# bodo-ai/Bodo

Measured on NVIDIA H100. Metric: groupby-agg rows/sec, higher is better.
Workload: dtype int64

## Files before the change

bodo_b200/csrc/groupby.cu:

```cuda
#include <algorithm>
#include <chrono>
#include <cmath>
#include <cstdio>
#include <cstdlib>
#include <cstring>
#include <type_traits>
#include <memory>
#include <vector>

#include <cooperative_groups.h>
#include <cooperative_groups/reduce.h>

#include "common.cuh"

namespace b200 {

constexpr long long EMPTY_KEY = (long long)0x8000000000000000ULL;
constexpr int MAX_OPS = 16;
constexpr int64_t CHUNK_ROWS = 1ll << 28;

enum OpKind : int { K_SUM_I64 = 0, K_SUM_F64, K_COUNT, K_SIZE, K_MEAN, K_MIN_I64, K_MAX_I64, K_MIN_F64, K_MAX_F64,
                    K_MOM2, K_MOM3,
                    K_FIRST, K_LAST,
                    K_NUNIQUE,
// ... 1522 lines not shown
    long long* retry_ctr;
    long long retry_cap;
    int sum_first;
    int ns;
    int n_pass;
    const long long* hot_tab;
    const int* n_hot;
    int reserve_tickets;
};
struct SpgDenseArgs : SpgArgs {
    long long kbase, vbase;
    unsigned int d_kb, d_vb;
    unsigned int d_mul, d_inv;
    unsigned int d_gmagic;
    int d_slots;
};

__device__ __forceinline__ uint64_t spg_hash(long long key) {
    uint64_t x = (uint64_t)key;
    return (x ^ (x >> 29)) * 0x9E3779B97F4A7C15ULL;
}
__device__ __forceinline__ unsigned int spg_owner(uint64_t h, int n_owners) { return __umulhi((unsigned int)(h >> 32), (unsigned int)n_owners); }
__device__ __forceinline__ unsigned int spg_slot(uint64_t h, int ns) { return __umulhi((unsigned int)(h >> 20), (unsigned int)ns); }

template <bool HAS_SUM, bool HAS_CNT>
__device__ __forceinline__ void spg_retry_row(const SpgArgs& a, long long key, unsigned long long sum, unsigned long long cnt) {
    unsigned long long f = atomicAdd((unsigned long long*)a.retry_ctr, 1ull);
    if (f >= (unsigned long long)a.retry_cap) { a.counters[CTR_RETRY_OVERFLOW] = 1; return; }
    unsigned long long* r = a.retry + f * 4;
    r[0] = (unsigned long long)key; r[1] = 1ull;
// ... 111 lines not shown
                 ::"r"(smem_u32(smem_dst)), "l"(gsrc), "r"(bytes), "r"(smem_u32(bar)) : "memory");
}

template <int TILE, int MAX_C, int ROW_BYTES, int TAIL>
struct SpgTileSmem {
    static constexpr size_t raw_k = 0, raw_v = raw_k + (size_t)TILE * 8, stage = raw_v + (size_t)TILE * 8;
    static constexpr size_t gbase = stage + (size_t)TILE * ROW_BYTES, mbar = gbase + (size_t)MAX_C * 8, hist = mbar + 16;
    static constexpr size_t lbase = hist + (size_t)MAX_C * 4, tail = lbase + (size_t)(MAX_C + 4) * 4, bytes = tail + TAIL;
    static_assert(stage % 16 == 0 && gbase % 16 == 0 && lbase % 16 == 0 && tail % 16 == 0, "K1 shared regions stay 16-byte aligned");
};

template <int TILE, int THREADS, typename Smem, typename LoadTma, typename LoadPartial, typename Init, typename Classify,
          typename Stage, typename OnRun, typename CopyOut>
__device__ __forceinline__ void spg_partition_tiles(unsigned char* smem, int64_t n_rows, int C, unsigned long long* cls_cnt,
                                                    LoadTma load_tma, LoadPartial load_partial, Init init, Classify classify,
                                                    Stage stage, OnRun on_run, CopyOut copy_out) {
    unsigned long long* gbase = (unsigned long long*)(smem + Smem::gbase);
    uint64_t* mbar = (uint64_t*)(smem + Smem::mbar);
    unsigned int* hist = (unsigned int*)(smem + Smem::hist);
    unsigned int* lbase = (unsigned int*)(smem + Smem::lbase);
    const int tid = threadIdx.x;
    constexpr int ROWS = TILE / THREADS;
    const int64_t n_tiles = (n_rows + TILE - 1) / TILE;
    if (tid == 0) {
        mbar_init(mbar, 1);
        asm volatile("fence.mbarrier_init.release.cluster;" ::: "memory");
        init();
    }
    for (int j = tid; j < C; j += THREADS) hist[j] = 0;
    __syncthreads();
    auto issue = [&](int64_t t) {
        const int64_t r0 = t * TILE;
        if (r0 + TILE <= n_rows && tid == 0) load_tma(r0, mbar);
    };
    uint32_t phase = 0;
    int64_t t = blockIdx.x;
    if (t < n_tiles) issue(t);
    for (; t < n_tiles; t += gridDim.x) {
        const int64_t r0 = t * TILE;
        const int64_t tn = t + gridDim.x;
        const bool full = r0 + TILE <= n_rows;
        if (full) {
            while (!mbar_try_wait(mbar, phase)) {}
            phase ^= 1;
        } else {
            load_partial(r0);
            __syncthreads();
        }
        int c[ROWS];
        unsigned int rk[ROWS];
        [[maybe_unused]] unsigned int w[ROWS];
#pragma unroll
        for (int r = 0; r < ROWS; r++) {
            const int j = r * THREADS + tid;
            c[r] = -1;
// ... 17 lines not shown
            }
            if (tid == 0) lbase[C] = carry;
        }
        __syncthreads();
#pragma unroll
        for (int r = 0; r < ROWS; r++) {
            if (c[r] < 0) continue;
            stage(lbase[c[r]] + rk[r], r * THREADS + tid, c[r], w[r]);
        }
        if (tid >= THREADS - C) {
            const int cl = tid - (THREADS - C);
            gbase[cl] = my_gbase - lbase[cl];
            on_run(cl, my_gbase, my_cnt);
        }
        __syncthreads();
        if (tn < n_tiles) issue(tn);
        copy_out(lbase[C]);
        for (int j = tid; j < C; j += THREADS) hist[j] = 0;
        __syncthreads();
    }
}

template <bool HOT>
using SpgK1Smem = SpgTileSmem<SPG_TILE, SPG_MAX_OWNERS, 16, SPG_TILE + (HOT ? SPG_HOT_SLOTS * 20 : 0)>;

template <bool HAS_SUM, bool HAS_CNT, bool HOT = false>
__global__ void __launch_bounds__(SPG_TTHREADS, SPG_TCTAS) spg_partition_tma_kernel(const __grid_constant__ SpgArgs a) {
    extern __shared__ __align__(128) unsigned char smem_tma_raw[];
    using L = SpgK1Smem<HOT>;
    long long* raw_k = (long long*)(smem_tma_raw + L::raw_k);
    long long* raw_v = (long long*)(smem_tma_raw + L::raw_v);
    longlong2* stage = (longlong2*)(smem_tma_raw + L::stage);
    const unsigned long long* gbase = (const unsigned long long*)(smem_tma_raw + L::gbase);
    unsigned char* stage_owner = smem_tma_raw + L::tail;
// ... 787 lines not shown
        {
            spgn_ns = ((int)(((size_t)max_smem - 256 - SPGN_QUEUE_BYTES) / 12) - SPG_STASH) & ~1;
            spgn_smem = (size_t)(spgn_ns + SPG_STASH) * 12 + SPGN_QUEUE_BYTES + 16;
            spgn_enabled = true;
            spgd_max_smem = (size_t)max_smem - 256;
            for_each_sum_cnt([&](auto s, auto c) {
                if (!set_smem_limit((const void*)spgn_partition_kernel<s, c>, SpgnK1Smem<false>::bytes)) spgn_enabled = false;
                if (!set_smem_limit((const void*)spgn_aggregate_kernel<s, c>, spgn_smem)) spgn_enabled = false;
                if (!set_smem_limit((const void*)spgn_partition_kernel<s, c, true>, SpgnK1Smem<true>::bytes)) spgd_max_smem = 0;
                if (!set_smem_limit((const void*)spgn_aggregate_kernel<s, c, true>, spgd_max_smem)) spgd_max_smem = 0;
            });
            const char* e8 = getenv("B200_SPG_NARROW");
            if (e8 && e8[0] == '0') spgn_enabled = false;
            const char* e9 = getenv("B200_SPG_DENSE");
            if ((e9 && e9[0] == '0') || !spgn_enabled || sms < 2) spgd_max_smem = 0;
        }
        {
            spgg_enabled = 2 * sms <= GEN_CLS;
            for_each_spgg_part([&](auto ks, auto vs) {
                if (!set_smem_limit((const void*)spgg_partition_kernel<ks, vs>, SpggK1Smem::bytes)) spgg_enabled = false;
            });
            for (int v = 0; v < 4; v++) {
                const int sb = 16 + ((v & 1) ? 16 : 0) + ((v & 2) ? 4 : 0);
                spgg_ns[v] = ((int)(((size_t)max_smem - 64) / sb) - SPG_STASH) & ~1;
                spgg_smem[v] = (size_t)(spgg_ns[v] + SPG_STASH) * sb + 16;
            }
            for_each_spgg_agg([&](auto s, auto mm, auto nn) {
                if (!set_smem_limit((const void*)spgg_aggregate_kernel<s, mm, nn>, spgg_smem[mm + 2 * nn])) spgg_enabled = false;
            });
            const char* e7 = getenv("B200_SPG_GEN");
            if (e7 && e7[0] == '0') spgg_enabled = false;
        }
        if (!set_smem_limit((const void*)spg_hot_sample_kernel, SPG_HOT_SAMPLE_SMEM)) return false;
        { const char* e4 = getenv("B200_SPG_HOT"); spg_hot_enabled = !(e4 && e4[0] == '0'); }
        d_hot.alloc((size_t)SPG_HOT_SLOTS * 8 + 48);
        { const char* e3 = getenv("B200_LC"); lc_enabled = !(e3 && e3[0] == '0'); }
        spg_owners = sms;
        d_bucket_cnt.alloc((size_t)(GEN_CLS + spg_owners) * SPG_CNT_STRIDE * 8);
        spg_state = 1;
        return true;
    }

    bool lc_enabled = true, lowcard_small = false;
    int spgn_ns = 0;
    size_t spgn_smem = 0;
    bool spgn_enabled = false;
    int spg_sample_wide = -1;
    int64_t spgn_launches = 0, spg16_launches = 0;
    size_t spgd_max_smem = 0;
    bool spgd_ok = false;
    long long spgd_kbase = 0, spgd_vbase = 0;
    unsigned int spgd_kb = 0, spgd_vb = 0;
    int spgd_slots = 0;
    int64_t spgd_wide_rows = 0, spgd_launches = 0;
    static constexpr unsigned int SPGD_MUL = 0x9E3779B1u;
    static unsigned int odd_inverse(unsigned int m) {
        unsigned int x = m;
        for (int i = 0; i < 4; i++) x *= 2u - m * x;
        return x;
    }
    void spgd_plan(long long kmin, long long kmax, long long vmin, long long vmax, bool has_vals) {
        spgd_ok = false;
        if (spgd_max_smem == 0 || kmin > kmax) return;
        const uint64_t range = (uint64_t)kmax - (uint64_t)kmin;
        if (range >= (1ull << 21)) return;
        const uint64_t pad = range / 32;
        long long kbase;
        if (kmin >= 0 && (uint64_t)kmin <= pad) kbase = 0;
        else if (kmin < LLONG_MIN + (long long)pad + 1) return;
// ... 28 lines not shown
    static constexpr int SPG_MAX_PASSES = 24;
    int spg_pass_count(int64_t est) const {
        int64_t p = (est + spg_group_capacity() - 1) / spg_group_capacity();
        return p <= 1 ? 1 : (p <= SPG_MAX_PASSES ? (int)p : 0);
    }
    bool lc_pick(int64_t est) { lowcard_small = est <= LC_SLOTS_SMALL / 4; return lc_enabled && est <= LC_SLOTS_BIG / 4; }
    int64_t spg_group_capacity() const { return (int64_t)spg_owners * (spg_ns * 7 / 10); }

    PooledBuf d_retry2[2];
    static constexpr int H_SPG_WORDS = 2 * N_COUNTERS + 5;
    long long* h_spg = nullptr;
    cudaEvent_t spg_ev[2] = {nullptr, nullptr};

    int64_t spgn_wide_rows = 0;
    static int spg_retry_slot(int slot) { return slot == 0 ? CTR_FAIL : CTR_RETRY1; }
    void spg_finish(int slot, int sum_j, int cnt_j) {
        B200_CUDA(cudaEventSynchronize(spg_ev[slot]));
        const long long* hc = h_spg + slot * N_COUNTERS;
        n_groups = hc[CTR_GROUPS];
        spgn_wide_rows = hc[CTR_WIDE];
        spgd_wide_rows = hc[CTR_DENSE_WIDE];
        const int64_t nr = hc[spg_retry_slot(slot)];
        if (nr == 0) return;
        spg_retry_rows += nr;
        B200_CUDA(cudaStreamSynchronize(stream));
        read_counters();
        B200_REQUIRE(h_counters[CTR_RETRY_OVERFLOW] == 0, "SM-partitioned groupby: a retry list overflowed its buffer (internal sizing error)");
        const int64_t pending = h_counters[CTR_FAIL] + h_counters[CTR_RETRY1];
        if (pending == 0) return;
        grow_to_fit(pending, (int64_t)spg_owners * spg_ns);
        for (int sl = 0; sl < 2; sl++) {
            int64_t cnt = h_counters[spg_retry_slot(sl)];
            if (cnt == 0) continue;
            B200_CUDA(cudaMemsetAsync((char*)d_counters.p + spg_retry_slot(sl) * 8, 0, 8, stream));
            CombineArgs c{};
            c.src = host_source(d_retry2[sl].p, &cnt, 1); c.row_words = 4;
            d_fail.ensure(device, (size_t)cnt * 4);
            c.fail_list = d_fail.as<uint32_t>(); c.n_ops = 0;
            int order[2] = {sum_j, cnt_j};
            if (sum_j >= 0 && cnt_j >= 0 && cnt_j < sum_j) std::swap(order[0], order[1]);
            if (order[0] < 0) std::swap(order[0], order[1]);
            for (int q = 0; q < 2; q++) if (order[q] >= 0) { c.kinds[c.n_ops] = K_SUM_I64; c.a0[c.n_ops] = d_a0[order[q]].p; c.a1[c.n_ops] = nullptr; c.n_ops++; }
            xchg_combine_kernel<<<grid_for(cnt), 256, 0, stream>>>(slot_table(), c);
            launches++;
            B200_CUDA(cudaGetLastError());
        }
        read_counters();
    }

    void consume_spg(const long long* keys, const long long* vals, int64_t n, int sum_j, int cnt_j, bool lowcard = false, int64_t est_groups = 0) {
        B200_REQUIRE(((uintptr_t)keys & 15) == 0 && ((uintptr_t)vals & 15) == 0, "SM-partitioned groupby: key and value columns must be 16-byte aligned");
        if (!h_spg) {
            h_spg = (long long*)pinned_acquire(H_SPG_WORDS * sizeof(long long));
            for (int b = 0; b < 2; b++) B200_CUDA(cudaEventCreateWithFlags(&spg_ev[b], cudaEventDisableTiming));
        }
        ScopedTimer timer{t_spg};
        read_counters();
        n_groups_bound = n_groups;
        if (!lowcard && !spg_hot_sampled) {
            int* d_nhot = (int*)(d_hot.as<long long>() + SPG_HOT_SLOTS);
            spg_hot_sample_kernel<<<1, 1024, SPG_HOT_SAMPLE_SMEM, stream>>>(keys, vals, n, d_hot.as<long long>(), d_nhot, d_hot.as<long long>() + SPG_HOT_SLOTS + 1);
            B200_CUDA(cudaMemcpyAsync(h_spg + 2 * N_COUNTERS, d_nhot, 5 * sizeof(long long), cudaMemcpyDeviceToHost, stream));
            B200_CUDA(cudaStreamSynchronize(stream));
            spg_n_hot = spg_hot_enabled ? ((int*)(h_spg + 2 * N_COUNTERS))[0] : 0;
            spg_sample_wide = ((int*)(h_spg + 2 * N_COUNTERS))[1];
            const long long* rng = h_spg + 2 * N_COUNTERS + 1;
            spgd_plan(rng[0], rng[1], rng[2], rng[3], vals != nullptr);
            spg_hot_sampled = true;
            launches++;
        }
        const bool narrow_sig = spgn_enabled && !lowcard && spg_n_hot == 0 && spg_sample_wide == 0;
        const int64_t launch_rows = narrow_sig ? 2 * SPG_LAUNCH_ROWS : SPG_LAUNCH_ROWS;
        int64_t li = 0;
        for (int64_t r0 = 0; r0 < n; r0 += launch_rows, li++) {
            int slot = (int)(li & 1);
            int64_t rows = std::min(launch_rows, n - r0);
            const int64_t bucket_cap = (rows / spg_owners) + (rows / spg_owners) / 8 + 4096;
            const bool small = lowcard_small;
            const int gl = (int)std::min<int64_t>((int64_t)sms * (small ? 3 : 2), (rows + LC_THREADS * 2 - 1) / (LC_THREADS * 2));
            const int g2 = (int)std::min<int64_t>((int64_t)sms * SPG_TCTAS, (rows + SPG_TILE - 1) / SPG_TILE);
            const bool hot = !lowcard && spg_hot_enabled && spg_n_hot > 0;
            const bool dense = narrow_sig && spgd_ok && spgd_wide_rows * 64 <= rows_consumed;
            const bool narrow = dense || (narrow_sig && spgn_wide_rows * 64 <= rows_consumed);
            const int64_t est_n = std::max<int64_t>(est_groups, 1);
            const int n_pass = dense ? 1 : narrow ? (int)std::min<int64_t>(SPG_MAX_PASSES, std::max<int64_t>(1, (est_n + spgn_group_capacity() - 1) / spgn_group_capacity()))
                                      : spg_passes;
            const int64_t retry_cap = rows + (lowcard ? (int64_t)gl * (small ? LC_SLOTS_SMALL : LC_SLOTS_BIG)
                                                      : (int64_t)spg_owners * ((narrow ? spgn_ns : spg_ns) + SPG_STASH) * n_pass
                                                        + (hot ? (int64_t)g2 * SPG_HOT_SLOTS : 0));
            double ta = now();
            d_bucket.ensure(device, (size_t)spg_owners * bucket_cap * 16);
            d_retry2[slot].ensure(device, (size_t)retry_cap * 32);
            t_alloc += now() - ta;
            B200_CUDA(cudaMemsetAsync(d_bucket_cnt.p, 0, (size_t)spg_owners * SPG_CNT_STRIDE * 8, stream));
            SpgArgs a{};
            a.keys = keys + r0; a.vals = vals ? vals + r0 : nullptr; a.n_rows = rows; a.n_owners = spg_owners;
            a.tkeys = d_keys.as<long long>(); a.cap = cap;
            a.acc_sum = sum_j >= 0 ? d_a0[sum_j].as<unsigned long long>() : nullptr;
            a.acc_cnt = cnt_j >= 0 ? d_a0[cnt_j].as<unsigned long long>() : nullptr;
            a.counters = d_counters.as<long long>(); a.group_limit = (long long)(cap / 2);
            a.retry_ctr = d_counters.as<long long>() + spg_retry_slot(slot);
            a.bucket = d_bucket.as<longlong2>(); a.bucket_cnt = d_bucket_cnt.as<unsigned long long>(); a.bucket_cap = bucket_cap;
            a.retry = d_retry2[slot].as<unsigned long long>(); a.retry_cap = retry_cap;
            a.sum_first = (sum_j >= 0 && cnt_j >= 0 && sum_j < cnt_j) ? 1 : 0; a.ns = spg_ns; a.n_pass = n_pass;
            const ProfEvents prof = prof_begin(profiling);
            if (lowcard) {
                size_t lsm = (size_t)(small ? LC_SLOTS_SMALL : LC_SLOTS_BIG) * 20 + 64;
                with_sum_cnt(sum_j >= 0, cnt_j >= 0, [&](auto s, auto c) {
                    if (small) groupby_lowcard_kernel<s, c, LC_SLOTS_SMALL, 3><<<gl, LC_THREADS, lsm, stream>>>(a);
                    else groupby_lowcard_kernel<s, c, LC_SLOTS_BIG, 2><<<gl, LC_THREADS, lsm, stream>>>(a);
                });
                lc_launches++;
            } else {
                if (hot) { a.hot_tab = d_hot.as<long long>(); a.n_hot = (const int*)(d_hot.as<long long>() + SPG_HOT_SLOTS); }
                if (narrow) {
                    a.ns = spgn_ns;
                    a.reserve_tickets = (n_groups_bound == 0 && li == 0 && est_groups > 0 && est_groups + est_groups / 4 <= (int64_t)(cap / 2)) ? 1 : 0;
                    a.bucket_cap = bucket_cap & ~1ll;
                    const int gn = (int)std::min<int64_t>((int64_t)sms * SPGN_CTAS, (rows + SPGN_TILE - 1) / SPGN_TILE);
                    if (dense) {
                        a.bucket_cap = bucket_cap & ~3ll;
                        SpgDenseArgs da{};
                        static_cast<SpgArgs&>(da) = a;
                        da.kbase = spgd_kbase; da.vbase = spgd_vbase; da.d_kb = spgd_kb; da.d_vb = spgd_vb;
                        da.d_mul = SPGD_MUL; da.d_inv = odd_inverse(SPGD_MUL);
                        da.d_gmagic = (unsigned int)((0xffffffffull + spg_owners) / spg_owners);
                        da.d_slots = spgd_slots;
                        const size_t dsm = (size_t)spgd_slots * 8;
                        with_sum_cnt(sum_j >= 0, cnt_j >= 0, [&](auto s, auto c) {
                            spgn_partition_kernel<s, c, true><<<gn, SPG_TTHREADS, SpgnK1Smem<true>::bytes, stream>>>(da);
                            spgn_aggregate_kernel<s, c, true><<<spg_owners, SPG_THREADS, dsm, stream>>>(da);
                        });
                        spgd_launches++;
                    } else {
                        with_sum_cnt(sum_j >= 0, cnt_j >= 0, [&](auto s, auto c) {
                            spgn_partition_kernel<s, c><<<gn, SPG_TTHREADS, SpgnK1Smem<false>::bytes, stream>>>(a);
                            spgn_aggregate_kernel<s, c><<<spg_owners, SPG_THREADS, spgn_smem, stream>>>(a);
                        });
                    }
                    spgn_launches++;
                } else {
                    with_sum_cnt(sum_j >= 0, cnt_j >= 0, [&](auto s, auto c) {
                        if (hot) spg_partition_tma_kernel<s, c, true><<<g2, SPG_TTHREADS, SpgK1Smem<true>::bytes, stream>>>(a);
                        else spg_partition_tma_kernel<s, c><<<g2, SPG_TTHREADS, SpgK1Smem<false>::bytes, stream>>>(a);
                        spg_aggregate_kernel<s, c><<<spg_owners, SPG_THREADS, spg_smem, stream>>>(a);
                    });
                    spg16_launches++;
                }
            }
            B200_CUDA(cudaGetLastError());
            prof_end(prof);
            B200_CUDA(cudaMemcpyAsync(h_spg + slot * N_COUNTERS, d_counters.p, N_COUNTERS * sizeof(long long), cudaMemcpyDeviceToHost, stream));
            B200_CUDA(cudaEventRecord(spg_ev[slot], stream));
            launches += 2; consume_launches++; spg_launches++;
            rows_consumed += rows;
            if (li > 0) spg_finish(1 - slot, sum_j, cnt_j);
        }
        if (li > 0) spg_finish((int)((li - 1) & 1), sum_j, cnt_j);
        read_counters();
        n_groups_bound = n_groups;
    }

    struct GenSig { int vcol = -1; bool has_sum = false, has_mm = false, has_nn = false; int layout = 0; };
    static bool gen_int_ok(int ct) { const int sz = ctype_size(ct); return (sz == 4 || sz == 8) && !ctype_is_float(ct) && ct != CT_UINT64; }
    bool gen_signature(const std::vector<const void*>& data, const std::vector<const uint8_t*>& valid, GenSig& gs) const {
        if (nk != 1 || n_funcs < 1 || n_funcs > GEN_MAX_F || !gen_int_ok(c_types[0])) return false;
        bool has_size = false;
        for (auto& f : funcs) {
            switch (f.kind) {
                case K_SIZE: has_size = true; continue;
                case K_COUNT: break;
                case K_SUM_I64: case K_MEAN: gs.has_sum = true; break;
                case K_MIN_I64: case K_MAX_I64: gs.has_mm = true; break;
// ... 62 lines not shown
                spgg_aggregate_kernel<s, m, nn><<<spg_owners, SPG_THREADS, spgg_smem[mm], stream>>>(g);
            });
            B200_CUDA(cudaGetLastError());
            prof_end(prof);
            launches += 2; consume_launches++; spg_launches++; spgg_launches++;
            rows_consumed += rows;
            settle<unsigned long long>(d_retry2[0], GEN_RETRY_WORDS, spg_retry_rows, [&](const unsigned long long* list, int64_t nr) {
                spgg_replay_kernel<<<grid_for(nr), 256, 0, stream>>>(make_args(), list, (long long)nr);
                launches++;
                B200_CUDA(cudaGetLastError());
            });
        }
        n_groups_bound = n_groups;
    }

    void consume_device_chunk(const std::vector<const void*>& data, const std::vector<const uint8_t*>& valid, int64_t n) {
        if (n == 0) return;
        if (nk > 1) { consume_mk(data, valid, n); return; }
        bool fast = c_types[0] == CT_INT64 && valid[0] == nullptr && n_funcs >= 1;
        int sum_j = -1, cnt_j = -1, vcol = -1;
        for (int j = 0; j < n_funcs && fast; j++) {
            const FuncSpec& f = funcs[j];
            if (f.kind == K_SUM_I64 && f.in_ctype == CT_INT64 && valid[f.in_col] == nullptr && sum_j < 0) {
                sum_j = j; vcol = f.in_col;
            } else if ((f.kind == K_SIZE || (f.kind == K_COUNT && !ctype_is_float(f.in_ctype) && valid[f.in_col] == nullptr)) && cnt_j < 0) {
                cnt_j = j;
            } else {
                fast = false;
            }
        }
        if (fast && (((uintptr_t)data[0] & 15) || (vcol >= 0 && ((uintptr_t)data[vcol] & 15)))) fast = false;
        const bool spg = n >= (1 << 20) && spg_probe();
        GenSig gs;
        const bool gen = !fast && spg && spgg_enabled && gen_signature(data, valid, gs);
        if (!(fast && spg) && !gen) { consume_direct(data, valid, n, fast, sum_j, cnt_j, vcol, false); return; }
        const char* env = getenv("B200_SPG");
        const bool force = fast && env && env[0] == '1';
        int64_t est = std::max(expected_groups_hint, n_groups);
        std::vector<const void*> d2(data); std::vector<const uint8_t*> v2(valid);
        int64_t left = n;
        const bool learned = !force && est == 0 && rows_consumed == 0;
        if (learned) {
            const int64_t prefix = std::min<int64_t>(n, 1 << 20);
            consume_direct(data, valid, prefix, fast, sum_j, cnt_j, vcol, true);
            est = n_groups;
            if (prefix == n) return;
            for (int c = 0; c < n_cols; c++) {
                if (data[c]) d2[c] = (const char*)data[c] + prefix * ctype_size(c_types[c]);
                if (valid[c]) v2[c] = valid[c] + prefix / 8;
            }
            left = n - prefix;
        }
        if (fast) {
            if (force || spg_pass_count(est) > 0) {
                spg_passes = std::max(1, spg_pass_count(est));
                const bool lowcard = (learned || est > 0) && lc_pick(est);
                consume_spg((const long long*)d2[0], vcol >= 0 ? (const long long*)d2[vcol] : nullptr, left, sum_j, cnt_j, lowcard, est);
                return;
            }
        } else if (est > LC_SLOTS_BIG / 4 && spgg_pass_count(est, gs.layout) > 0 && left >= (1 << 16)) {
            consume_spg_gen(d2, v2, left, gs, spgg_pass_count(est, gs.layout));
            return;
        }
        consume_direct(d2, v2, left, fast, sum_j, cnt_j, vcol, false);
    }

    void consume_direct(const std::vector<const void*>& data, const std::vector<const uint8_t*>& valid, int64_t n, bool fast, int sum_j,
                        int cnt_j, int vcol, bool force_count) {
        bool could_fail = force_count || (int64_t)(cap / 2) - n_groups_bound < n;
        if (could_fail) d_fail.ensure(device, (size_t)n * 4);
        auto launch = [&](const uint32_t* index_list, int64_t rows) {
            const ProfEvents prof = prof_begin(profiling && index_list == nullptr);
            if (fast && index_list == nullptr) {
                const long long* k = (const long long*)data[0];
                const long long* v = vcol >= 0 ? (const long long*)data[vcol] : nullptr;
                unsigned long long* as = sum_j >= 0 ? d_a0[sum_j].as<unsigned long long>() : nullptr;
                unsigned long long* ac = cnt_j >= 0 ? d_a0[cnt_j].as<unsigned long long>() : nullptr;
                with_sum_cnt(sum_j >= 0, cnt_j >= 0, [&](auto s, auto c) {
                    groupby_consume_i64_sumcount_kernel<s, c><<<grid_for(rows, 2), 256, 0, stream>>>(
// ... 515 lines not shown
            if (!used[c]) continue;
            B200_REQUIRE(t->cols[c].c_type == in_types[c], "b200 groupby: batch column dtype differs from the build schema");
            B200_REQUIRE(n == 0 || t->cols[c].data != nullptr, "b200 groupby: null data pointer");
        }
        for (auto& ni : nu_inner) {
            b200_column pc[2] = {t->cols[0], t->cols[ni.in_col]};
            b200_table pt{};
            pt.n_cols = 2; pt.n_rows = n; pt.cols = pc; pt.device = t->device;
            ni.st->consume(&pt);
            B200_CUDA(cudaSetDevice(device)); scratch_set_stream(stream);
        }
        if (coalesce(t, n)) return;
        flush_coalesced();
        if (t->device >= 0) {
            B200_REQUIRE(t->device == device, "b200 groupby: batch lives on a different device than the state");
            for (int64_t r0 = 0; r0 < n; r0 += CHUNK_ROWS) {
                int64_t rows = std::min(CHUNK_ROWS, n - r0);
                B200_REQUIRE(r0 % 8 == 0, "internal: chunk offset must be byte aligned for validity bitmaps");
                std::vector<const void*> data(n_cols, nullptr);
                std::vector<const uint8_t*> valid(n_cols, nullptr);
                for (int c = 0; c < n_cols; c++) {
                    if (!used[c]) continue;
                    data[c] = (const char*)t->cols[c].data + r0 * ctype_size(in_types[c]);
                    valid[c] = t->cols[c].validity ? t->cols[c].validity + r0 / 8 : nullptr;
                }
                consume_chunk(data, valid, rows);
            }
            return;
        }
        const int64_t HCHUNK = 1ll << 24;
        if (!copy_stream) {
            B200_CUDA(cudaStreamCreateWithFlags(&copy_stream, cudaStreamNonBlocking));
// ... 497 lines not shown
        case 6: return (int64_t)s->consume_kernel_us();
        case 7: return s->consume_launches;
        case 8: return s->spg_launches;
        case 9: return s->spg_retry_rows;
        case 10: return s->lc_launches;
        case 11: return s->co_batches;
        case 12: return s->spgg_launches;
        case 14: return s->spgn_launches;
        case 15: return s->spg16_launches;
        case 16: return s->spg_n_hot;
        case 17: return s->spgd_launches;
        case 18: return s->mt.admitted;
        case 19: return s->mt.reduces;
        case 20: { cudaSetDevice(s->device); return s->ho.on ? s->holistic_rows() : 0; }
        case 21: return s->ho.passes;
        case 13: { cudaSetDevice(s->device); s->read_counters(); return s->n_groups; }
        case 100: s->profiling = true; return 0;
        default: return -1;
    }
}

}
```

bodo_b200/csrc/spgn.cuh:

```cuda
#pragma once

#ifndef SPGN_TILE_ROWS
#define SPGN_TILE_ROWS 4096
#endif
constexpr int SPGN_TILE = SPGN_TILE_ROWS;
constexpr int SPGN_CTAS = SPGN_TILE == 4096 ? 2 : 3;
constexpr int SPGN_QUEUE = 32;
constexpr int SPGN_QUEUE_BYTES = SPG_THREADS / 32 * SPGN_QUEUE * 9;

__device__ __forceinline__ uint64_t spgn_insert_ticketed(long long* __restrict__ tkeys, uint64_t cap, long long key, bool& inserted) {
    const uint64_t mask = cap - 1;
    uint64_t s = (key_hash(key) >> 32) & mask;
    inserted = false;
    while (true) {
        long long k = __ldcg(tkeys + s);
        if (k == EMPTY_KEY) {
            k = (long long)atomicCAS((unsigned long long*)(tkeys + s), (unsigned long long)EMPTY_KEY, (unsigned long long)key);
            if (k == EMPTY_KEY) { inserted = true; return s; }
        }
        if (k == key) return s;
        s = (s + 1) & mask;
    }
}

// ... 13 lines not shown
template <bool HAS_SUM, bool HAS_CNT, bool DENSE = false>
__global__ void __launch_bounds__(SPG_TTHREADS, SPGN_CTAS) spgn_partition_kernel(const __grid_constant__ std::conditional_t<DENSE, SpgDenseArgs, SpgArgs> a) {
    using Row = std::conditional_t<DENSE, unsigned int, int2>;
    using L = SpgnK1Smem<DENSE>;
    extern __shared__ __align__(128) unsigned char smem_n_raw[];
    long long* raw_k = (long long*)(smem_n_raw + L::raw_k);
    long long* raw_v = (long long*)(smem_n_raw + L::raw_v);
    Row* stage = (Row*)(smem_n_raw + L::stage);
    const unsigned long long* gbase = (const unsigned long long*)(smem_n_raw + L::gbase);
    unsigned char* stage_owner = smem_n_raw + L::tail;
    Row** dptr = (Row**)(stage_owner + SPGN_TILE);
    unsigned int* tile_over = (unsigned int*)(dptr + SPG_MAX_OWNERS);
    const int G = a.n_owners, tid = threadIdx.x;
    Row* bucket = reinterpret_cast<Row*>(a.bucket);
    unsigned int wide = 0;
    spg_partition_tiles<SPGN_TILE, SPG_TTHREADS, L>(
        smem_n_raw, a.n_rows, G, a.bucket_cnt,
        [&](int64_t r0, uint64_t* mbar) {
            mbar_expect_tx(mbar, (HAS_SUM ? 2u : 1u) * SPGN_TILE * 8u);
            tma_load_1d(raw_k, a.keys + r0, SPGN_TILE * 8u, mbar);
            if (HAS_SUM) tma_load_1d(raw_v, a.vals + r0, SPGN_TILE * 8u, mbar);
        },
        [&](int64_t r0) {
            for (int j = tid; j < SPGN_TILE; j += SPG_TTHREADS) {
                int64_t i = r0 + j;
                raw_k[j] = i < a.n_rows ? a.keys[i] : 0;
                raw_v[j] = (HAS_SUM && i < a.n_rows) ? a.vals[i] : 0;
            }
        },
        [&] { *tile_over = 0; },
// ... 36 lines not shown
                if (p < n_tile) dptr[stage_owner[p]][p] = stage[p];
            } else {
                for (unsigned int p = tid; p < n_tile; p += SPG_TTHREADS) {
                    const unsigned int ow = stage_owner[p];
                    const unsigned long long off = gbase[ow] + p;
                    const Row row = stage[p];
                    if (off < (unsigned long long)a.bucket_cap) bucket[(size_t)ow * a.bucket_cap + off] = row;
                    else if constexpr (DENSE)
                        spg_direct_apply<HAS_SUM, HAS_CNT>(a, spgd_key(a, row >> a.d_vb, ow),
                                                           (unsigned long long)a.vbase + (row & ((1u << a.d_vb) - 1u)), 1ull);
                    else spg_direct_apply<HAS_SUM, HAS_CNT>(a, (long long)row.x, (unsigned long long)(long long)row.y, 1ull);
                }
            }
            __syncthreads();
            if (tid == 0) *tile_over = 0;
        });
    if (wide) atomicAdd((unsigned long long*)&a.counters[DENSE ? CTR_DENSE_WIDE : CTR_WIDE], (unsigned long long)wide);
}

template <bool HAS_SUM, bool HAS_CNT>
__device__ __noinline__ void spgn_cold_row(const SpgArgs& a, int* skeys, unsigned int* slo, unsigned int* scnt, unsigned int NB, int key, int val,
                                           bool added) {
    unsigned int old = 0;
    if (!added) {
        const int s = spg_claim(skeys, 2 * NB, spg_hash((long long)key), key);
        if (s < 0) { spg_direct_apply<HAS_SUM, HAS_CNT>(a, (long long)key, (unsigned long long)(long long)val, 1ull); return; }
        if (HAS_SUM) old = atomicAdd(&slo[s], (unsigned int)val);
        if (HAS_CNT) atomicAdd(&scnt[s], 1u);
    }
    if (HAS_SUM) {
        const unsigned int lo = (unsigned int)val;
        const unsigned int hi = added ? (val < 0 ? 0xffffffffu : 1u) : (val < 0 ? 0xffffffffu : 0u) + (old + lo < old ? 1u : 0u);
// ... 4 lines not shown
#ifdef SPGN_PHASE_CLOCKS
__device__ unsigned long long spgn_phase_clocks[SPG_MAX_OWNERS * 4];
#define SPGN_PHASE(i)                                                                                                      \
    do {                                                                                                                   \
        if (threadIdx.x == 0) {                                                                                            \
            unsigned long long* c_ = spgn_phase_clocks + blockIdx.x * 4;                                                   \
            const unsigned long long t_ = clock64();                                                                       \
            if ((i) >= 0) c_[(i)] += t_ - c_[3];                                                                           \
            c_[3] = t_;                                                                                                    \
        }                                                                                                                  \
    } while (0)
#else
#define SPGN_PHASE(i) do {} while (0)
#endif

template <bool HAS_SUM, bool HAS_CNT, typename Occupied, typename Entry>
__device__ __forceinline__ void spg_flush_ticketed(const SpgArgs& a, int n_slots, Occupied occupied, Entry entry) {
    const int tid = threadIdx.x;
    __shared__ unsigned int fl_occ, fl_dup;
    __shared__ int fl_reserved;
    if (tid == 0) { fl_occ = 0; fl_dup = 0; fl_reserved = 0; }
    __syncthreads();
    if (a.reserve_tickets && a.group_limit >= 0) {
        unsigned int mine = 0;
        for (int s = tid; s < n_slots; s += SPG_THREADS) mine += occupied(s);
        for (int d = 16; d; d >>= 1) mine += __shfl_xor_sync(0xffffffffu, mine, d);
        if ((tid & 31) == 0 && mine) atomicAdd(&fl_occ, mine);
        __syncthreads();
        if (tid == 0 && fl_occ) {
            const long long t = (long long)atomicAdd((unsigned long long*)&a.counters[CTR_GROUPS], (unsigned long long)fl_occ);
            if (t + (long long)fl_occ <= a.group_limit) fl_reserved = 1;
            else atomicAdd((unsigned long long*)&a.counters[CTR_GROUPS], (unsigned long long)(-(long long)fl_occ));
        }
        __syncthreads();
    }
    const bool reserved = fl_reserved != 0;
    unsigned int dup = 0;
    for (int s = tid; s < n_slots; s += SPG_THREADS) {
        if (!occupied(s)) continue;
        long long key;
        unsigned long long sum, cnt;
        entry(s, key, sum, cnt);
        if (!reserved) { spg_direct_apply<HAS_SUM, HAS_CNT>(a, key, sum, cnt); continue; }
        bool inserted;
        const uint64_t sl = spgn_insert_ticketed(a.tkeys, a.cap, key, inserted);
        if (!inserted) dup++;
        if (HAS_SUM && sum) atomicAdd(a.acc_sum + sl, sum);
        if (HAS_CNT && cnt) atomicAdd(a.acc_cnt + sl, cnt);
    }
    if (reserved) {
        for (int d = 16; d; d >>= 1) dup += __shfl_xor_sync(0xffffffffu, dup, d);
        if ((tid & 31) == 0 && dup) atomicAdd(&fl_dup, dup);
        __syncthreads();
// ... 110 lines not shown
        __syncthreads();
        SPGN_PHASE(1);
#ifdef SPGN_SKIP_FLUSH
        continue;
#endif
        spg_flush_ticketed<HAS_SUM, HAS_CNT>(a, NT, [&](int s) { return skeys[s] != SPGN_EMPTY; },
                                             [&](int s, long long& key, unsigned long long& sum, unsigned long long& cnt) {
                                                 key = (long long)skeys[s];
                                                 sum = (unsigned long long)slo[s] - 0x80000000ull;
                                                 cnt = (unsigned long long)scnt[s];
                                             });
        SPGN_PHASE(2);
    }
}

template <bool HAS_SUM, bool HAS_CNT>
__device__ __noinline__ void spgd_carry(const SpgDenseArgs& a, unsigned int slot) {
    spg_direct_apply<HAS_SUM, HAS_CNT>(a, spgd_key(a, slot, blockIdx.x), 1ull << 32, 0ull);
}

template <bool HAS_SUM, bool HAS_CNT>
__device__ __forceinline__ void spgd_aggregate(const SpgDenseArgs& a) {
    extern __shared__ __align__(16) unsigned char smem_raw[];
    const int NS = a.d_slots, tid = threadIdx.x, me = blockIdx.x;
    unsigned int* ssum = (unsigned int*)smem_raw;
    unsigned int* scnt = ssum + NS;
    for (int s = tid; s < NS; s += SPG_THREADS) { ssum[s] = 0; scnt[s] = 0; }
    __syncthreads();
    unsigned long long n_in = a.bucket_cnt[me * SPG_CNT_STRIDE];
    if (n_in > (unsigned long long)a.bucket_cap) n_in = (unsigned long long)a.bucket_cap;
    const unsigned int* src = reinterpret_cast<const unsigned int*>(a.bucket) + (size_t)me * a.bucket_cap;
    const unsigned int vb = a.d_vb, vmask = (1u << vb) - 1u;
    auto add = [&](unsigned int w) {
        const unsigned int s = w >> vb;
        if (HAS_SUM) {
            const unsigned int e = w & vmask, old = atomicAdd(&ssum[s], e);
            if (old + e < old) spgd_carry<HAS_SUM, HAS_CNT>(a, s);
        }
        atomicAdd(&scnt[s], 1u);
    };
    constexpr int V = 2;
    const uint4* src4 = reinterpret_cast<const uint4*>(src);
    const unsigned long long n4 = n_in / 4, step = (unsigned long long)V * SPG_THREADS, full = n4 / step * step;
    if (full > 0) {
        uint4 cur[V], nxt[V];
#pragma unroll
        for (int j = 0; j < V; j++) cur[j] = __ldcs(src4 + tid + j * SPG_THREADS);
        for (unsigned long long ub = 0; ub < full; ub += step) {
            if (ub + step < full) {
#pragma unroll
                for (int j = 0; j < V; j++) nxt[j] = __ldcs(src4 + ub + step + tid + j * SPG_THREADS);
            }
#pragma unroll
            for (int j = 0; j < V; j++) { add(cur[j].x); add(cur[j].y); add(cur[j].z); add(cur[j].w); }
#pragma unroll
            for (int j = 0; j < V; j++) cur[j] = nxt[j];
        }
    }
    for (unsigned long long i = 4 * full + tid; i < n_in; i += SPG_THREADS) add(__ldcs(src + i));
    __syncthreads();
    const unsigned long long vbase = (unsigned long long)a.vbase;
    spg_flush_ticketed<HAS_SUM, HAS_CNT>(a, NS, [&](int s) { return scnt[s] != 0; },
                                 [&](int s, long long& key, unsigned long long& sum, unsigned long long& cnt) {
                                     cnt = (unsigned long long)scnt[s];
                                     key = spgd_key(a, (unsigned int)s, (unsigned int)me);
                                     sum = (unsigned long long)ssum[s] + cnt * vbase;
                                 });
}

template <bool HAS_SUM, bool HAS_CNT, bool DENSE = false>
__global__ void __launch_bounds__(SPG_THREADS, 1) spgn_aggregate_kernel(const __grid_constant__ std::conditional_t<DENSE, SpgDenseArgs, SpgArgs> a) {
    if constexpr (DENSE) spgd_aggregate<HAS_SUM, HAS_CNT>(a);
    else spgn_hash_aggregate<HAS_SUM, HAS_CNT>(a);
}
```

Measured before the change: 108.3 billion.

## Overlap dense partition and aggregate kernels across launches with PDL and ticketed tiles

Uses programmatic dependent launch so the next chunk's dense partition kernel can start while the previous aggregate kernel is still running. Partition CTAs claim tiles dynamically through an atomic ticket, and the bucket buffers and count blocks are double-buffered so the two launches do not collide; the aggregate kernel resets counts itself to avoid memsets. It also retunes the dense aggregate to 512 threads with two CTAs per SM and deeper load prefetch, skips chunking for fast-signature batches, and defers the counter snapshot so the host sync does not stall the pipeline. This adds risk around shared-memory and register co-residency and more complex retry and counter handling.

```diff
diff --git a/bodo_b200/csrc/groupby.cu b/bodo_b200/csrc/groupby.cu
--- a/bodo_b200/csrc/groupby.cu
+++ b/bodo_b200/csrc/groupby.cu
@@ -1560,6 +1560,7 @@
     unsigned int d_mul, d_inv;
     unsigned int d_gmagic;
     int d_slots;
+    unsigned long long* tile_ticket;
 };
 
 __device__ __forceinline__ uint64_t spg_hash(long long key) {
@@ -1701,7 +1702,8 @@
           typename Stage, typename OnRun, typename CopyOut>
 __device__ __forceinline__ void spg_partition_tiles(unsigned char* smem, int64_t n_rows, int C, unsigned long long* cls_cnt,
                                                     LoadTma load_tma, LoadPartial load_partial, Init init, Classify classify,
-                                                    Stage stage, OnRun on_run, CopyOut copy_out) {
+                                                    Stage stage, OnRun on_run, CopyOut copy_out, unsigned long long* ticket = nullptr) {
+    __shared__ long long next_ticket;
     unsigned long long* gbase = (unsigned long long*)(smem + Smem::gbase);
     uint64_t* mbar = (uint64_t*)(smem + Smem::mbar);
     unsigned int* hist = (unsigned int*)(smem + Smem::hist);
@@ -1723,9 +1725,9 @@
     uint32_t phase = 0;
     int64_t t = blockIdx.x;
     if (t < n_tiles) issue(t);
-    for (; t < n_tiles; t += gridDim.x) {
+    while (t < n_tiles) {
         const int64_t r0 = t * TILE;
-        const int64_t tn = t + gridDim.x;
+        if (ticket && tid == 0) next_ticket = (long long)gridDim.x + (long long)atomicAdd(ticket, 1ull);
         const bool full = r0 + TILE <= n_rows;
         if (full) {
             while (!mbar_try_wait(mbar, phase)) {}
@@ -1773,10 +1775,12 @@
             on_run(cl, my_gbase, my_cnt);
         }
         __syncthreads();
+        const int64_t tn = ticket ? (int64_t)next_ticket : t + gridDim.x;
         if (tn < n_tiles) issue(tn);
         copy_out(lbase[C]);
         for (int j = tid; j < C; j += THREADS) hist[j] = 0;
         __syncthreads();
+        t = tn;
     }
 }
 
@@ -2594,6 +2598,30 @@
             if (e8 && e8[0] == '0') spgn_enabled = false;
             const char* e9 = getenv("B200_SPG_DENSE");
             if ((e9 && e9[0] == '0') || !spgn_enabled || sms < 2) spgd_max_smem = 0;
+            const char* e10 = getenv("B200_SPG_OVERLAP");
+            int regs_sm = 0, smem_sm = 0, smem_rsv = 0;
+            cudaDeviceGetAttribute(&regs_sm, cudaDevAttrMaxRegistersPerMultiprocessor, device);
+            cudaDeviceGetAttribute(&smem_sm, cudaDevAttrMaxSharedMemoryPerMultiprocessor, device);
+            cudaDeviceGetAttribute(&smem_rsv, cudaDevAttrReservedSharedMemoryPerBlock, device);
+            int regs = 0;
+            size_t static_smem = 0;
+            for_each_sum_cnt([&](auto s, auto c) {
+                cudaFuncAttributes f1{}, f2{};
+                B200_CUDA(cudaFuncGetAttributes(&f1, (const void*)spgn_partition_kernel<s, c, true>));
+                B200_CUDA(cudaFuncGetAttributes(&f2, (const void*)spgn_aggregate_kernel<s, c, true>));
+                auto warp_regs = [](int r) { return (r * 32 + 255) / 256 * 256; };
+                regs = std::max(regs, warp_regs(f1.numRegs) * (SPG_TTHREADS / 32) + warp_regs(f2.numRegs) * (SPGD_THREADS / 32));
+                static_smem = std::max(static_smem, f1.sharedSizeBytes + f2.sharedSizeBytes);
+            });
+            spgd_overlap_smem = 0;
+            if (!(e10 && e10[0] == '0') && spgd_max_smem > 0 && regs <= regs_sm && SPG_TTHREADS + SPGD_THREADS <= 2048) {
+                const size_t fixed = SpgnK1Smem<true>::bytes + static_smem + 2 * (size_t)smem_rsv;
+                if (fixed < (size_t)smem_sm) spgd_overlap_smem = (size_t)smem_sm - fixed;
+                for_each_sum_cnt([&](auto s, auto c) {
+                    B200_CUDA(cudaFuncSetAttribute((const void*)spgn_partition_kernel<s, c, true>, cudaFuncAttributePreferredSharedMemoryCarveout, cudaSharedmemCarveoutMaxShared));
+                    B200_CUDA(cudaFuncSetAttribute((const void*)spgn_aggregate_kernel<s, c, true>, cudaFuncAttributePreferredSharedMemoryCarveout, cudaSharedmemCarveoutMaxShared));
+                });
+            }
         }
         {
             spgg_enabled = 2 * sms <= GEN_CLS;
@@ -2616,7 +2644,7 @@
         d_hot.alloc((size_t)SPG_HOT_SLOTS * 8 + 48);
         { const char* e3 = getenv("B200_LC"); lc_enabled = !(e3 && e3[0] == '0'); }
         spg_owners = sms;
-        d_bucket_cnt.alloc((size_t)(GEN_CLS + spg_owners) * SPG_CNT_STRIDE * 8);
+        d_bucket_cnt.alloc((size_t)std::max(GEN_CLS + spg_owners, 2 * (spg_owners + 1)) * SPG_CNT_STRIDE * 8);
         spg_state = 1;
         return true;
     }
@@ -2633,6 +2661,14 @@
     unsigned int spgd_kb = 0, spgd_vb = 0;
     int spgd_slots = 0;
     int64_t spgd_wide_rows = 0, spgd_launches = 0;
+    PooledBuf d_bucket2;
+    size_t spgd_overlap_smem = 0;
+    int64_t spgd_overlap_launches = 0;
+    bool spgd_cnt_dirty[2] = {true, true};
+    bool spgd_prev_overlap = false;
+    unsigned long long* spgd_cnt_block(int par) const {
+        return d_bucket_cnt.as<unsigned long long>() + (size_t)par * (spg_owners + 1) * SPG_CNT_STRIDE;
+    }
     static constexpr unsigned int SPGD_MUL = 0x9E3779B1u;
     static unsigned int odd_inverse(unsigned int m) {
         unsigned int x = m;
@@ -2691,20 +2727,20 @@
 
     int64_t spgn_wide_rows = 0;
     static int spg_retry_slot(int slot) { return slot == 0 ? CTR_FAIL : CTR_RETRY1; }
-    void spg_finish(int slot, int sum_j, int cnt_j) {
+    bool spg_finish(int slot, int sum_j, int cnt_j) {
         B200_CUDA(cudaEventSynchronize(spg_ev[slot]));
         const long long* hc = h_spg + slot * N_COUNTERS;
         n_groups = hc[CTR_GROUPS];
         spgn_wide_rows = hc[CTR_WIDE];
         spgd_wide_rows = hc[CTR_DENSE_WIDE];
         const int64_t nr = hc[spg_retry_slot(slot)];
-        if (nr == 0) return;
-        spg_retry_rows += nr;
+        if (nr == 0) return false;
         B200_CUDA(cudaStreamSynchronize(stream));
         read_counters();
         B200_REQUIRE(h_counters[CTR_RETRY_OVERFLOW] == 0, "SM-partitioned groupby: a retry list overflowed its buffer (internal sizing error)");
         const int64_t pending = h_counters[CTR_FAIL] + h_counters[CTR_RETRY1];
-        if (pending == 0) return;
+        if (pending == 0) return false;
+        spg_retry_rows += pending;
         grow_to_fit(pending, (int64_t)spg_owners * spg_ns);
         for (int sl = 0; sl < 2; sl++) {
             int64_t cnt = h_counters[spg_retry_slot(sl)];
@@ -2723,6 +2759,7 @@
             B200_CUDA(cudaGetLastError());
         }
         read_counters();
+        return true;
     }
 
     void consume_spg(const long long* keys, const long long* vals, int64_t n, int sum_j, int cnt_j, bool lowcard = false, int64_t est_groups = 0) {
@@ -2748,6 +2785,9 @@
         }
         const bool narrow_sig = spgn_enabled && !lowcard && spg_n_hot == 0 && spg_sample_wide == 0;
         const int64_t launch_rows = narrow_sig ? 2 * SPG_LAUNCH_ROWS : SPG_LAUNCH_ROWS;
+        B200_CUDA(cudaMemsetAsync(spgd_cnt_block(0), 0, (size_t)2 * (spg_owners + 1) * SPG_CNT_STRIDE * 8, stream));
+        spgd_cnt_dirty[0] = spgd_cnt_dirty[1] = false;
+        spgd_prev_overlap = false;
         int64_t li = 0;
         for (int64_t r0 = 0; r0 < n; r0 += launch_rows, li++) {
             int slot = (int)(li & 1);
@@ -2765,11 +2805,19 @@
             const int64_t retry_cap = rows + (lowcard ? (int64_t)gl * (small ? LC_SLOTS_SMALL : LC_SLOTS_BIG)
                                                       : (int64_t)spg_owners * ((narrow ? spgn_ns : spg_ns) + SPG_STASH) * n_pass
                                                         + (hot ? (int64_t)g2 * SPG_HOT_SLOTS : 0));
+            const bool overlap = dense && (size_t)spgd_slots * 8 <= spgd_overlap_smem;
             double ta = now();
-            d_bucket.ensure(device, (size_t)spg_owners * bucket_cap * 16);
+            if (dense && slot == 1) d_bucket2.ensure(device, (size_t)spg_owners * bucket_cap * 4);
+            else d_bucket.ensure(device, (size_t)spg_owners * bucket_cap * 16);
             d_retry2[slot].ensure(device, (size_t)retry_cap * 32);
             t_alloc += now() - ta;
-            B200_CUDA(cudaMemsetAsync(d_bucket_cnt.p, 0, (size_t)spg_owners * SPG_CNT_STRIDE * 8, stream));
+            const int blk = dense ? slot : 0;
+            bool cleared = false;
+            if (!dense || spgd_cnt_dirty[blk]) {
+                B200_CUDA(cudaMemsetAsync(spgd_cnt_block(blk), 0, (size_t)(spg_owners + 1) * SPG_CNT_STRIDE * 8, stream));
+                cleared = true;
+            }
+            spgd_cnt_dirty[blk] = !dense;
             SpgArgs a{};
             a.keys = keys + r0; a.vals = vals ? vals + r0 : nullptr; a.n_rows = rows; a.n_owners = spg_owners;
             a.tkeys = d_keys.as<long long>(); a.cap = cap;
@@ -2777,12 +2825,18 @@
             a.acc_cnt = cnt_j >= 0 ? d_a0[cnt_j].as<unsigned long long>() : nullptr;
             a.counters = d_counters.as<long long>(); a.group_limit = (long long)(cap / 2);
             a.retry_ctr = d_counters.as<long long>() + spg_retry_slot(slot);
-            a.bucket = d_bucket.as<longlong2>(); a.bucket_cnt = d_bucket_cnt.as<unsigned long long>(); a.bucket_cap = bucket_cap;
+            a.bucket = d_bucket.as<longlong2>(); a.bucket_cnt = spgd_cnt_block(blk); a.bucket_cap = bucket_cap;
             a.retry = d_retry2[slot].as<unsigned long long>(); a.retry_cap = retry_cap;
             a.sum_first = (sum_j >= 0 && cnt_j >= 0 && sum_j < cnt_j) ? 1 : 0; a.ns = spg_ns; a.n_pass = n_pass;
             const ProfEvents prof = prof_begin(profiling);
+            auto snapshot_prev = [&] {
+                if (li == 0) return;
+                B200_CUDA(cudaMemcpyAsync(h_spg + (1 - slot) * N_COUNTERS, d_counters.p, N_COUNTERS * sizeof(long long), cudaMemcpyDeviceToHost, stream));
+                B200_CUDA(cudaEventRecord(spg_ev[1 - slot], stream));
+            };
             if (lowcard) {
                 size_t lsm = (size_t)(small ? LC_SLOTS_SMALL : LC_SLOTS_BIG) * 20 + 64;
+                snapshot_prev();
                 with_sum_cnt(sum_j >= 0, cnt_j >= 0, [&](auto s, auto c) {
                     if (small) groupby_lowcard_kernel<s, c, LC_SLOTS_SMALL, 3><<<gl, LC_THREADS, lsm, stream>>>(a);
                     else groupby_lowcard_kernel<s, c, LC_SLOTS_BIG, 2><<<gl, LC_THREADS, lsm, stream>>>(a);
@@ -2797,21 +2851,37 @@
                     const int gn = (int)std::min<int64_t>((int64_t)sms * SPGN_CTAS, (rows + SPGN_TILE - 1) / SPGN_TILE);
                     if (dense) {
                         a.bucket_cap = bucket_cap & ~3ll;
+                        if (slot == 1) a.bucket = d_bucket2.as<longlong2>();
                         SpgDenseArgs da{};
                         static_cast<SpgArgs&>(da) = a;
                         da.kbase = spgd_kbase; da.vbase = spgd_vbase; da.d_kb = spgd_kb; da.d_vb = spgd_vb;
                         da.d_mul = SPGD_MUL; da.d_inv = odd_inverse(SPGD_MUL);
                         da.d_gmagic = (unsigned int)((0xffffffffull + spg_owners) / spg_owners);
                         da.d_slots = spgd_slots;
+                        da.tile_ticket = spgd_cnt_block(blk) + (size_t)spg_owners * SPG_CNT_STRIDE;
                         const size_t dsm = (size_t)spgd_slots * 8;
+                        const bool pdl = overlap && spgd_prev_overlap && !cleared && !profiling;
                         with_sum_cnt(sum_j >= 0, cnt_j >= 0, [&](auto s, auto c) {
-                            spgn_partition_kernel<s, c, true><<<gn, SPG_TTHREADS, SpgnK1Smem<true>::bytes, stream>>>(da);
-                            spgn_aggregate_kernel<s, c, true><<<spg_owners, SPG_THREADS, dsm, stream>>>(da);
+                            if (pdl) {
+                                cudaLaunchAttribute at[1];
+                                at[0].id = cudaLaunchAttributeProgrammaticStreamSerialization;
+                                at[0].val.programmaticStreamSerializationAllowed = 1;
+                                cudaLaunchConfig_t cfg{};
+                                cfg.gridDim = dim3(gn); cfg.blockDim = dim3(SPG_TTHREADS); cfg.dynamicSmemBytes = SpgnK1Smem<true>::bytes;
+                                cfg.stream = stream; cfg.attrs = at; cfg.numAttrs = 1;
+                                B200_CUDA(cudaLaunchKernelEx(&cfg, spgn_partition_kernel<s, c, true>, da));
+                            } else {
+                                spgn_partition_kernel<s, c, true><<<gn, SPG_TTHREADS, SpgnK1Smem<true>::bytes, stream>>>(da);
+                            }
+                            snapshot_prev();
+                            spgn_aggregate_kernel<s, c, true><<<spg_owners, SPGD_THREADS, dsm, stream>>>(da);
                         });
                         spgd_launches++;
+                        spgd_overlap_launches += pdl;
                     } else {
                         with_sum_cnt(sum_j >= 0, cnt_j >= 0, [&](auto s, auto c) {
                             spgn_partition_kernel<s, c><<<gn, SPG_TTHREADS, SpgnK1Smem<false>::bytes, stream>>>(a);
+                            snapshot_prev();
                             spgn_aggregate_kernel<s, c><<<spg_owners, SPG_THREADS, spgn_smem, stream>>>(a);
                         });
                     }
@@ -2820,6 +2890,7 @@
                     with_sum_cnt(sum_j >= 0, cnt_j >= 0, [&](auto s, auto c) {
                         if (hot) spg_partition_tma_kernel<s, c, true><<<g2, SPG_TTHREADS, SpgK1Smem<true>::bytes, stream>>>(a);
                         else spg_partition_tma_kernel<s, c><<<g2, SPG_TTHREADS, SpgK1Smem<false>::bytes, stream>>>(a);
+                        snapshot_prev();
                         spg_aggregate_kernel<s, c><<<spg_owners, SPG_THREADS, spg_smem, stream>>>(a);
                     });
                     spg16_launches++;
@@ -2827,13 +2898,17 @@
             }
             B200_CUDA(cudaGetLastError());
             prof_end(prof);
-            B200_CUDA(cudaMemcpyAsync(h_spg + slot * N_COUNTERS, d_counters.p, N_COUNTERS * sizeof(long long), cudaMemcpyDeviceToHost, stream));
-            B200_CUDA(cudaEventRecord(spg_ev[slot], stream));
             launches += 2; consume_launches++; spg_launches++;
             rows_consumed += rows;
-            if (li > 0) spg_finish(1 - slot, sum_j, cnt_j);
-        }
-        if (li > 0) spg_finish((int)((li - 1) & 1), sum_j, cnt_j);
+            const bool enqueued = li > 0 && spg_finish(1 - slot, sum_j, cnt_j);
+            spgd_prev_overlap = overlap && !enqueued;
+        }
+        if (li > 0) {
+            const int last = (int)((li - 1) & 1);
+            B200_CUDA(cudaMemcpyAsync(h_spg + last * N_COUNTERS, d_counters.p, N_COUNTERS * sizeof(long long), cudaMemcpyDeviceToHost, stream));
+            B200_CUDA(cudaEventRecord(spg_ev[last], stream));
+            spg_finish(last, sum_j, cnt_j);
+        }
         read_counters();
         n_groups_bound = n_groups;
     }
@@ -2926,11 +3001,9 @@
         n_groups_bound = n_groups;
     }
 
-    void consume_device_chunk(const std::vector<const void*>& data, const std::vector<const uint8_t*>& valid, int64_t n) {
-        if (n == 0) return;
-        if (nk > 1) { consume_mk(data, valid, n); return; }
-        bool fast = c_types[0] == CT_INT64 && valid[0] == nullptr && n_funcs >= 1;
-        int sum_j = -1, cnt_j = -1, vcol = -1;
+    bool fast_signature(const std::vector<const void*>& data, const std::vector<const uint8_t*>& valid, int& sum_j, int& cnt_j, int& vcol) const {
+        bool fast = nk == 1 && c_types[0] == CT_INT64 && valid[0] == nullptr && n_funcs >= 1;
+        sum_j = cnt_j = vcol = -1;
         for (int j = 0; j < n_funcs && fast; j++) {
             const FuncSpec& f = funcs[j];
             if (f.kind == K_SUM_I64 && f.in_ctype == CT_INT64 && valid[f.in_col] == nullptr && sum_j < 0) {
@@ -2941,11 +3014,18 @@
                 fast = false;
             }
         }
-        if (fast && (((uintptr_t)data[0] & 15) || (vcol >= 0 && ((uintptr_t)data[vcol] & 15)))) fast = false;
+        return fast && !((uintptr_t)data[0] & 15) && !(vcol >= 0 && ((uintptr_t)data[vcol] & 15));
+    }
+
+    void consume_device_chunk(const std::vector<const void*>& data, const std::vector<const uint8_t*>& valid, int64_t n) {
+        if (n == 0) return;
+        if (nk > 1) { consume_mk(data, valid, n); return; }
+        int sum_j, cnt_j, vcol;
+        const bool fast = fast_signature(data, valid, sum_j, cnt_j, vcol);
         const bool spg = n >= (1 << 20) && spg_probe();
         GenSig gs;
         const bool gen = !fast && spg && spgg_enabled && gen_signature(data, valid, gs);
-        if (!(fast && spg) && !gen) { consume_direct(data, valid, n, fast, sum_j, cnt_j, vcol, false); return; }
+        if (!(fast && spg) && !gen) { consume_direct_chunks(data, valid, n, fast, sum_j, cnt_j, vcol); return; }
         const char* env = getenv("B200_SPG");
         const bool force = fast && env && env[0] == '1';
         int64_t est = std::max(expected_groups_hint, n_groups);
@@ -2974,7 +3054,20 @@
             consume_spg_gen(d2, v2, left, gs, spgg_pass_count(est, gs.layout));
             return;
         }
-        consume_direct(d2, v2, left, fast, sum_j, cnt_j, vcol, false);
+        consume_direct_chunks(d2, v2, left, fast, sum_j, cnt_j, vcol);
+    }
+
+    void consume_direct_chunks(const std::vector<const void*>& data, const std::vector<const uint8_t*>& valid, int64_t n, bool fast, int sum_j,
+                               int cnt_j, int vcol) {
+        std::vector<const void*> d(data);
+        std::vector<const uint8_t*> v(valid);
+        for (int64_t r0 = 0; r0 < n; r0 += CHUNK_ROWS) {
+            for (int c = 0; c < n_cols; c++) {
+                if (data[c]) d[c] = (const char*)data[c] + r0 * ctype_size(c_types[c]);
+                if (valid[c]) v[c] = valid[c] + r0 / 8;
+            }
+            consume_direct(d, v, std::min(CHUNK_ROWS, n - r0), fast, sum_j, cnt_j, vcol, false);
+        }
     }
 
     void consume_direct(const std::vector<const void*>& data, const std::vector<const uint8_t*>& valid, int64_t n, bool fast, int sum_j,
@@ -3520,8 +3613,16 @@
         flush_coalesced();
         if (t->device >= 0) {
             B200_REQUIRE(t->device == device, "b200 groupby: batch lives on a different device than the state");
-            for (int64_t r0 = 0; r0 < n; r0 += CHUNK_ROWS) {
-                int64_t rows = std::min(CHUNK_ROWS, n - r0);
+            int64_t chunk = CHUNK_ROWS;
+            if (!mr.on && !ho.on && nk == 1 && !float_key(0)) {
+                std::vector<const void*> d0(n_cols, nullptr);
+                std::vector<const uint8_t*> v0(n_cols, nullptr);
+                for (int c = 0; c < n_cols; c++) if (used[c]) { d0[c] = t->cols[c].data; v0[c] = t->cols[c].validity; }
+                int sj, cj, vc;
+                if (fast_signature(d0, v0, sj, cj, vc)) chunk = std::max<int64_t>(n, 1);
+            }
+            for (int64_t r0 = 0; r0 < n; r0 += chunk) {
+                int64_t rows = std::min(chunk, n - r0);
                 B200_REQUIRE(r0 % 8 == 0, "internal: chunk offset must be byte aligned for validity bitmaps");
                 std::vector<const void*> data(n_cols, nullptr);
                 std::vector<const uint8_t*> valid(n_cols, nullptr);
@@ -4049,6 +4150,7 @@
         case 19: return s->mt.reduces;
         case 20: { cudaSetDevice(s->device); return s->ho.on ? s->holistic_rows() : 0; }
         case 21: return s->ho.passes;
+        case 22: return s->spgd_overlap_launches;
         case 13: { cudaSetDevice(s->device); s->read_counters(); return s->n_groups; }
         case 100: s->profiling = true; return 0;
         default: return -1;
diff --git a/bodo_b200/csrc/spgn.cuh b/bodo_b200/csrc/spgn.cuh
--- a/bodo_b200/csrc/spgn.cuh
+++ b/bodo_b200/csrc/spgn.cuh
@@ -51,6 +51,8 @@
     const int G = a.n_owners, tid = threadIdx.x;
     Row* bucket = reinterpret_cast<Row*>(a.bucket);
     unsigned int wide = 0;
+    unsigned long long* ticket = nullptr;
+    if constexpr (DENSE) ticket = a.tile_ticket;
     spg_partition_tiles<SPGN_TILE, SPG_TTHREADS, L>(
         smem_n_raw, a.n_rows, G, a.bucket_cnt,
         [&](int64_t r0, uint64_t* mbar) {
@@ -117,8 +119,10 @@
             }
             __syncthreads();
             if (tid == 0) *tile_over = 0;
-        });
+        },
+        ticket);
     if (wide) atomicAdd((unsigned long long*)&a.counters[DENSE ? CTR_DENSE_WIDE : CTR_WIDE], (unsigned long long)wide);
+    if constexpr (DENSE) asm volatile("griddepcontrol.wait;" ::: "memory");
 }
 
 template <bool HAS_SUM, bool HAS_CNT>
@@ -153,7 +157,7 @@
 #define SPGN_PHASE(i) do {} while (0)
 #endif
 
-template <bool HAS_SUM, bool HAS_CNT, typename Occupied, typename Entry>
+template <bool HAS_SUM, bool HAS_CNT, int THREADS = SPG_THREADS, typename Occupied, typename Entry>
 __device__ __forceinline__ void spg_flush_ticketed(const SpgArgs& a, int n_slots, Occupied occupied, Entry entry) {
     const int tid = threadIdx.x;
     __shared__ unsigned int fl_occ, fl_dup;
@@ -162,7 +166,7 @@
     __syncthreads();
     if (a.reserve_tickets && a.group_limit >= 0) {
         unsigned int mine = 0;
-        for (int s = tid; s < n_slots; s += SPG_THREADS) mine += occupied(s);
+        for (int s = tid; s < n_slots; s += THREADS) mine += occupied(s);
         for (int d = 16; d; d >>= 1) mine += __shfl_xor_sync(0xffffffffu, mine, d);
         if ((tid & 31) == 0 && mine) atomicAdd(&fl_occ, mine);
         __syncthreads();
@@ -175,7 +179,7 @@
     }
     const bool reserved = fl_reserved != 0;
     unsigned int dup = 0;
-    for (int s = tid; s < n_slots; s += SPG_THREADS) {
+    for (int s = tid; s < n_slots; s += THREADS) {
         if (!occupied(s)) continue;
         long long key;
         unsigned long long sum, cnt;
@@ -316,6 +320,7 @@
     }
 }
 
+constexpr int SPGD_THREADS = 512;
 template <bool HAS_SUM, bool HAS_CNT>
 __device__ __noinline__ void spgd_carry(const SpgDenseArgs& a, unsigned int slot) {
     spg_direct_apply<HAS_SUM, HAS_CNT>(a, spgd_key(a, slot, blockIdx.x), 1ull << 32, 0ull);
@@ -324,12 +329,18 @@
 template <bool HAS_SUM, bool HAS_CNT>
 __device__ __forceinline__ void spgd_aggregate(const SpgDenseArgs& a) {
     extern __shared__ __align__(16) unsigned char smem_raw[];
+    constexpr int T = SPGD_THREADS;
     const int NS = a.d_slots, tid = threadIdx.x, me = blockIdx.x;
     unsigned int* ssum = (unsigned int*)smem_raw;
     unsigned int* scnt = ssum + NS;
-    for (int s = tid; s < NS; s += SPG_THREADS) { ssum[s] = 0; scnt[s] = 0; }
+    unsigned long long n_in = a.bucket_cnt[me * SPG_CNT_STRIDE];
+    for (int s = tid; s < NS; s += T) { ssum[s] = 0; scnt[s] = 0; }
     __syncthreads();
-    unsigned long long n_in = a.bucket_cnt[me * SPG_CNT_STRIDE];
+    if (tid == 0) {
+        a.bucket_cnt[me * SPG_CNT_STRIDE] = 0;
+        if (me == 0) *a.tile_ticket = 0;
+    }
+    asm volatile("griddepcontrol.launch_dependents;" ::: "memory");
     if (n_in > (unsigned long long)a.bucket_cap) n_in = (unsigned long long)a.bucket_cap;
     const unsigned int* src = reinterpret_cast<const unsigned int*>(a.bucket) + (size_t)me * a.bucket_cap;
     const unsigned int vb = a.d_vb, vmask = (1u << vb) - 1u;
@@ -341,17 +352,17 @@
         }
         atomicAdd(&scnt[s], 1u);
     };
-    constexpr int V = 2;
+    constexpr int V = 3;
     const uint4* src4 = reinterpret_cast<const uint4*>(src);
-    const unsigned long long n4 = n_in / 4, step = (unsigned long long)V * SPG_THREADS, full = n4 / step * step;
+    const unsigned long long n4 = n_in / 4, step = (unsigned long long)V * T, full = n4 / step * step;
     if (full > 0) {
         uint4 cur[V], nxt[V];
 #pragma unroll
-        for (int j = 0; j < V; j++) cur[j] = __ldcs(src4 + tid + j * SPG_THREADS);
+        for (int j = 0; j < V; j++) cur[j] = __ldcs(src4 + tid + j * T);
         for (unsigned long long ub = 0; ub < full; ub += step) {
             if (ub + step < full) {
 #pragma unroll
-                for (int j = 0; j < V; j++) nxt[j] = __ldcs(src4 + ub + step + tid + j * SPG_THREADS);
+                for (int j = 0; j < V; j++) nxt[j] = __ldcs(src4 + ub + step + tid + j * T);
             }
 #pragma unroll
             for (int j = 0; j < V; j++) { add(cur[j].x); add(cur[j].y); add(cur[j].z); add(cur[j].w); }
@@ -359,10 +370,10 @@
             for (int j = 0; j < V; j++) cur[j] = nxt[j];
         }
     }
-    for (unsigned long long i = 4 * full + tid; i < n_in; i += SPG_THREADS) add(__ldcs(src + i));
+    for (unsigned long long i = 4 * full + tid; i < n_in; i += T) add(__ldcs(src + i));
     __syncthreads();
     const unsigned long long vbase = (unsigned long long)a.vbase;
-    spg_flush_ticketed<HAS_SUM, HAS_CNT>(a, NS, [&](int s) { return scnt[s] != 0; },
+    spg_flush_ticketed<HAS_SUM, HAS_CNT, T>(a, NS, [&](int s) { return scnt[s] != 0; },
                                  [&](int s, long long& key, unsigned long long& sum, unsigned long long& cnt) {
                                      cnt = (unsigned long long)scnt[s];
                                      key = spgd_key(a, (unsigned int)s, (unsigned int)me);
@@ -371,7 +382,7 @@
 }
 
 template <bool HAS_SUM, bool HAS_CNT, bool DENSE = false>
-__global__ void __launch_bounds__(SPG_THREADS, 1) spgn_aggregate_kernel(const __grid_constant__ std::conditional_t<DENSE, SpgDenseArgs, SpgArgs> a) {
+__global__ void __launch_bounds__(DENSE ? SPGD_THREADS : SPG_THREADS, DENSE ? 2 : 1) spgn_aggregate_kernel(const __grid_constant__ std::conditional_t<DENSE, SpgDenseArgs, SpgArgs> a) {
     if constexpr (DENSE) spgd_aggregate<HAS_SUM, HAS_CNT>(a);
     else spgn_hash_aggregate<HAS_SUM, HAS_CNT>(a);
 }
```

Result: no change. 109.2 billion, median of 6 (+0.9%).
